# Metronlab/bow

Measured on AMD Instinct MI355X. Metric: rows/sec rolling-mean on 1B-row float64, higher is better.
Workload: dtype f64; 1 GPU; IntervalRolling(interval=10, offset=0)+Aggregate(WindowStart,ArithmeticMean), dense int64 ts=i + float64 u01 values, 1000000000 rows/GPU resident in HBM, null_count=0; rows_per_gpu=1000000000, windows_per_gpu=100000000, parallelism=rows range-partitioned x1

## Files before the change

### bow_amd/capi.py

```python
import contextlib
import ctypes as C
import os

import numpy as np

_HERE = os.path.dirname(os.path.abspath(__file__))
LIB_PATH = os.environ.get("BOWGPU_LIB") or os.path.join(_HERE, "libbowgpu.so")

FLOAT64, INT64, BOOLEAN, STRING = 1, 2, 3, 4
HOST, DEVICE, HOST_PINNED = 0, 1, 2
TYPE_NAMES = {"float64": FLOAT64, "int64": INT64, "bool": BOOLEAN, "utf8": STRING}

AGG = {
    "WindowStart": 0, "Sum": 1, "ArithmeticMean": 2, "Min": 3, "Max": 4, "Count": 5, "First": 6,
    "Last": 7, "IntegralStep": 8, "IntegralTrapezoid": 9, "WeightedAverageStep": 10,
    "WeightedAverageLinear": 11, "NumRows": 12, "Mode": 13,
}
INTERP = {"WindowStart": 0, "Linear": 1, "StepPrevious": 2, "None": 3, "Const": 4}

MAX_FACTORS = 4
CARRY_MAX_AGGS = 16
ABI_VERSION = 7

ERR_NAMES = {
# ... 146 lines not shown
    n = C.c_int(0)
    arr = (C.c_int * 64)()
    check(lib().bowgpu_get_devices(arr, 64, C.byref(n)))
    return [arr[i] for i in range(n.value)]


def fanout_counts():
    a, b = C.c_int64(0), C.c_int64(0)
    check(lib().bowgpu_fanout_counts(C.byref(a), C.byref(b)))
    return a.value, b.value


def last_call_ranks():
    n = C.c_int(0)
    check(lib().bowgpu_last_call_ranks(C.byref(n)))
    return n.value


class devices:

    def __init__(self, ids, min_rows=None):
        self.ids, self.min_rows = list(ids), min_rows

    def __enter__(self):
        self.prev = get_devices()
        set_devices(self.ids, self.min_rows)
        return self

    def __exit__(self, *exc):
        set_devices(self.prev, (1 << 20) if self.min_rows is not None else None)
        return False


def mem_info():
    f, t = C.c_int64(0), C.c_int64(0)
    check(lib().bowgpu_mem_info(C.byref(f), C.byref(t)))
    return f.value, t.value


def trim(all_threads=True):
    n = C.c_int64(0)
    check(lib().bowgpu_trim(1 if all_threads else 0, C.byref(n)))
    return n.value


def check(rc):
    if rc != 0:
        raise BowGpuError(rc, lib().bowgpu_last_error().decode("utf-8", "replace"))


ROUTE_NO_SIMPLE, ROUTE_FORCE_GENERAL, ROUTE_NO_LONG_ONLY, ROUTE_LONG_CLASSIC, ROUTE_LONG_STREAM_ALL = 1, 2, 4, 8, 16
ROUTE_SIMPLE_SMALL_LIST, ROUTE_SIMPLE_LARGE_LIST, ROUTE_TW_F64, ROUTE_SIMPLE_PADDED, ROUTE_INTERP_TILE = 32, 64, 128, 256, 512
ROUTE_PINNED_STAGE, ROUTE_STRICT_ORDER, ROUTE_NO_FUSED, ROUTE_TW_ROWS, ROUTE_INTERP_COPIES = 1024, 2048, 4096, 8192, 16384
ROUTE_QUEUE_HOST, ROUTE_QUEUE_DEVICE = 32768, 65536


def set_route(mask):
    check(lib().bowgpu_debug_set_route(C.c_uint32(mask)))


def get_route():
    m = C.c_uint32(0)
    check(lib().bowgpu_debug_get_route(C.byref(m)))
    return m.value


class route:

    def __init__(self, mask):
        self.mask = mask

    def __enter__(self):
        self.prev = get_route()
        set_route(self.mask)
        return self

    def __exit__(self, *exc):
        set_route(self.prev)
        return False


AGG_ROUTES = (("auto", 0), ("classic-long", ROUTE_LONG_CLASSIC), ("stream-all", ROUTE_LONG_STREAM_ALL),
              ("small-list", ROUTE_SIMPLE_SMALL_LIST), ("large-list", ROUTE_SIMPLE_LARGE_LIST), ("padded", ROUTE_SIMPLE_PADDED), ("tw-rows", ROUTE_TW_ROWS),
              ("queue-device", ROUTE_NO_LONG_ONLY | ROUTE_QUEUE_DEVICE), ("queue-host", ROUTE_NO_LONG_ONLY | ROUTE_QUEUE_HOST),
              ("lean", ROUTE_NO_SIMPLE | ROUTE_NO_LONG_ONLY), ("general", ROUTE_FORCE_GENERAL | ROUTE_NO_LONG_ONLY))
INTERP_ROUTES = (("wave3", 0), ("tile", ROUTE_INTERP_TILE))


def agg_routes():
    for label, mask in AGG_ROUTES:
        with route(mask):
            yield label


class DeviceBuffer:

    def __init__(self, nbytes):
        self.nbytes = int(nbytes)
        p = C.c_void_p()
        check(lib().bowgpu_malloc(C.byref(p), C.c_int64(self.nbytes)))
        self.ptr = p.value

    @classmethod
    def from_numpy(cls, arr):
        arr = np.ascontiguousarray(arr)
        b = cls(max(arr.nbytes, 8))
        if arr.nbytes:
# ... 520 lines not shown
```

### bow_amd/csrc/api.cpp

```cpp

#include <stdarg.h>
#include <stdio.h>
#include <stdlib.h>
#include <string.h>
#include <time.h>
#include <execinfo.h>
#include <signal.h>
#include <unistd.h>

#include <algorithm>
#include <atomic>
#include <condition_variable>
#include <mutex>
#include <thread>
#include <vector>

#include "common.h"

namespace bowgpu {

static thread_local char g_err[512] = "";

void set_error(const char *fmt, ...) {
    va_list ap;
// ... 600 lines not shown
    case BOWGPU_AGG_FIRST:
    case BOWGPU_AGG_LAST: return BOWGPU_INPUT_DEPENDENT;
    case BOWGPU_AGG_MODE: return BOWGPU_INPUT_DEPENDENT;
    default: return BOWGPU_FLOAT64;
    }
}

bool kind_never_nil(int kind) {
    return kind == BOWGPU_AGG_WINDOW_START || kind == BOWGPU_AGG_SUM || kind == BOWGPU_AGG_COUNT || kind == BOWGPU_AGG_NUM_ROWS;
}

bool kind_reads_values(int kind) { return !(kind == BOWGPU_AGG_WINDOW_START || kind == BOWGPU_AGG_NUM_ROWS); }

struct AggRun {
    Plan plan;
    std::vector<DevCol> dcols;
    std::vector<DevOut> douts;
    AggParams params;
    int inclusive = 0;
    int new_interval_col = -1;
};

static int validate_aggs(const bowgpu_col *cols, int32_t ncols, int32_t ts_col, const bowgpu_agg *aggs, int32_t naggs,
                         int *inclusive, int *new_interval_col) {
    if (naggs <= 0) return fail(BOWGPU_ERR_NO_AGG, "at least one column aggregation is required");
    int nic = -1;
    for (int i = 0; i < naggs; i++) {
        if (aggs[i].col < 0 || aggs[i].col >= ncols) return fail(BOWGPU_ERR_BAD_COL, "aggregation %d: no column with index %d", i, aggs[i].col);
        if (aggs[i].kind < 0 || aggs[i].kind >= BOWGPU_AGG__COUNT) return fail(BOWGPU_ERR_ARG, "aggregation %d: unknown kind %d", i, aggs[i].kind);
        if (aggs[i].n_factors < 0 || aggs[i].n_factors > BOWGPU_MAX_FACTORS) return fail(BOWGPU_ERR_ARG, "aggregation %d: bad factor count", i);
        const int t = cols[aggs[i].col].type;
        if (t != BOWGPU_FLOAT64 && t != BOWGPU_INT64)
            return fail(BOWGPU_ERR_UNSUPPORTED, "aggregation %d: column type %d is outside the device path (Float64/Int64 only)", i, t);
        if (kind_needs_inclusive(aggs[i].kind)) *inclusive = 1;
        if (aggs[i].col == ts_col) nic = i;
    }
    if (nic == -1) return fail(BOWGPU_ERR_KEEP_INTERVAL, "must keep interval column");
    *new_interval_col = nic;
    return 0;
}

struct AggJob {
    std::vector<DevCol> dcols;
    std::vector<DevOut> douts;
    DevCol dts;
    AggParams P;
    int64_t W = 0;
    size_t scratch_bytes = 0;
    int inclusive = 0;
    bool counts_used = false;
    bool tail_wrote_host = false;
    bool check_plan = false;
    bool band_rows = false;
};
static thread_local bool g_plan_from_caller = false;
static int64_t compact_long_max_rows(const bowgpu_agg *aggs, int32_t naggs) {
    bool step = false, trap = false, mm = false, fl = false;
    for (int i = 0; i < naggs; i++) {
        const int k = aggs[i].kind;
        step |= k == BOWGPU_AGG_INTEGRAL_STEP || k == BOWGPU_AGG_WAVG_STEP;
        trap |= k == BOWGPU_AGG_INTEGRAL_TRAPEZOID || k == BOWGPU_AGG_WAVG_LINEAR;
        mm |= k == BOWGPU_AGG_MIN || k == BOWGPU_AGG_MAX;
        fl |= k == BOWGPU_AGG_FIRST || k == BOWGPU_AGG_LAST;
    }
    if ((step && trap) || mm) return kCompactLongBothMaxAvgRows;
    if (step || trap || fl) return kCompactLongMaxAvgRows;
    return 0;
}
static thread_local bool g_strict_order = false;

static void pending_drop(Ctx *c);

static int job_build(Ctx *c, const bowgpu_col *cols, int32_t ncols, int32_t ts_col, const Plan &plan, int inclusive,
                     const bowgpu_agg *aggs, int32_t naggs, bowgpu_out *outs, int64_t wid_base, int64_t W,
                     bool holds_row0, AggJob *job, int nullable_per_pass = 4) {
    pending_drop(c);
    const bowgpu_col *tsc = &cols[ts_col];
    const int64_t n = tsc->length;
    for (int i = 0; i < ncols; i++)
        if (cols[i].length != n) return fail(BOWGPU_ERR_ARG, "column %d has %lld rows, interval column has %lld", i, (long long)cols[i].length, (long long)n);

    if (tsc->validity && tsc->null_count != 0) {
        DevCol probe;
        BG_TRY(devcol_prepare(c, tsc, &probe, false, true));
        if (probe.null_count > 0)
            return fail(BOWGPU_ERR_TS_NULLS, "interval column has %lld nulls: outside the device path", (long long)probe.null_count);
    }

    job->dcols.clear();
    job->dcols.resize(ncols);
    job->douts.clear();
    job->douts.resize(naggs);
    job->W = W;
    job->inclusive = inclusive;
    job->check_plan = g_plan_from_caller;
    std::vector<DevCol> &dcols = job->dcols;
    std::vector<int> slot_of(ncols, -1);
    AggParams &P = job->P;
    memset(&P, 0, sizeof P);
    {
        bowgpu_col t = *tsc;
        t.validity = nullptr;
        t.null_count = 0;
        BG_TRY(devcol_prepare(c, &t, &job->dts, true, false));
    }
    P.ts = reinterpret_cast<const int64_t *>(job->dts.values);
// ... 61 lines not shown
        BG_TRY(devout_prepare(c, &outs[i], W, &job->douts[i], i));
        a.out_values = job->douts[i].values;
        a.out_valid = kind_never_nil(aggs[i].kind) ? nullptr : reinterpret_cast<uint32_t *>(job->douts[i].validity);
    }

    P.first_pass_slot = kMaxCols;
    P.last_val_slot = -1;
    for (int i = 0; i < naggs; i++) {
        const AggDesc &d = P.aggs[i];
        const int k = d.kind;
        const int idx = d.slot + 1;
        P.pass_mask[idx] |= 1u << i;
        uint32_t fl = 0;
        if (kind_reads_values(k)) fl |= kPassNeedVals;
        if (k == BOWGPU_AGG_MIN || k == BOWGPU_AGG_MAX) fl |= kPassMinMax;
        if (k == BOWGPU_AGG_FIRST || k == BOWGPU_AGG_LAST) fl |= kPassFirstLast;
        if (d.out_valid) fl |= kPassNullable;
        if (k >= BOWGPU_AGG_INTEGRAL_STEP && k <= BOWGPU_AGG_WAVG_LINEAR && d.slot >= 0) P.cols[d.slot].need_ts = 1;
        P.pass_flags[idx] |= fl;
        if (d.slot < P.first_pass_slot) P.first_pass_slot = d.slot;
        if (kind_reads_values(k) && d.slot > P.last_val_slot) P.last_val_slot = d.slot;
    }
    for (int s = 0; s <= kMaxCols; s++) {
        int nn = 0;
        for (int i = 0; i < naggs; i++) if ((P.pass_mask[s] >> i) & 1u) nn += P.aggs[i].out_valid != nullptr;
        if (nn > P.n_nullable_max) P.n_nullable_max = nn;
    }

    const int64_t ntiles = (n + 511) / 512;
    const int64_t sub_cap = ntiles / kLongLists + 2;
    job->scratch_bytes = 8192 + (size_t)sub_cap * kLongLists * 16;
    void *dscr;
    BG_TRY(ctx_scratch(c, job->scratch_bytes, &dscr));
    P.status = reinterpret_cast<uint32_t *>(dscr);
    P.long_list = reinterpret_cast<int64_t *>(reinterpret_cast<char *>(dscr) + 8192);
    P.long_cap = sub_cap;
    return 0;
}

constexpr size_t kCountsOffset = 1024;
constexpr size_t kReadbackBytes = kCountsOffset + 8 * kMaxAggs;
static_assert(kStatusWords * 4 <= kCountsOffset, "status words overlap the counters");

static void job_bitmaps(AggJob *job, const bowgpu_agg *aggs, int32_t naggs, bool all_ones, BitmapBatch *b) {
    memset(b, 0, sizeof *b);
    b->n = naggs;
    b->status_words = kStatusWords;
    b->nbits = job->W > 0 ? job->W : 0;
    b->status = job->P.status;
    b->counts = reinterpret_cast<unsigned long long *>(reinterpret_cast<char *>(job->P.status) + kCountsOffset);
    for (int i = 0; i < naggs; i++) {
        b->work[i] = reinterpret_cast<uint32_t *>(job->douts[i].validity);
        const bowgpu_out *u = job->douts[i].user;
        b->user[i] = (u && u->residency == BOWGPU_DEVICE) ? u->validity : nullptr;
        b->ones[i] = all_ones || kind_never_nil(aggs[i].kind);
        b->count[i] = !kind_never_nil(aggs[i].kind);
    }
}

static int job_enqueue_tail(Ctx *c, AggJob *job, const bowgpu_agg *aggs, int32_t naggs) {
    const int64_t W = job->W;
    if (W > 0) {
        BitmapBatch b;
        job_bitmaps(job, aggs, naggs, false, &b);
        if (W <= kFinishHostBits) {
            BG_TRY(ctx_pinned(c, 16384, reinterpret_cast<void **>(&b.host_block)));
            job->tail_wrote_host = true;
        } else if (job->counts_used) BG_HIP(hipMemsetAsync(b.counts, 0, 8 * kMaxAggs, c->stream));
        BG_TRY(launch_finish_bitmaps(c, b));
        job->counts_used = true;
    }
    for (int i = 0; i < naggs; i++) BG_TRY(devout_finish(c, &job->douts[i], W, job->P.aggs[i].out_type, 0, false));
    return 0;
}

static int job_readback(Ctx *c, AggJob *job, uint32_t **hstat, uint64_t **hcnt) {
    char *hp;
    BG_TRY(ctx_pinned(c, 16384, reinterpret_cast<void **>(&hp)));
    if (job->tail_wrote_host) job->tail_wrote_host = false;
    else BG_HIP(hipMemcpyAsync(hp, job->P.status, kReadbackBytes, hipMemcpyDeviceToHost, c->stream));
    *hstat = reinterpret_cast<uint32_t *>(hp);
    *hcnt = reinterpret_cast<uint64_t *>(hp + kCountsOffset);
    return 0;
}

static bool simple_applies(const AggJob *job, const bowgpu_agg *aggs, int32_t naggs, const Plan &plan, bool time_weighted, int *need,
                           bool *is_int, bool *has_nulls, bool *wide) {
    const AggParams &P = job->P;
    if ((job->inclusive && !time_weighted) || !P.fits32 || naggs > kSimpleMaxAggs) return false;
    if (P.W <= 0) return false;

    const int64_t slot0_start = P.s0 + (int64_t)((uint64_t)P.wid_base * (uint64_t)P.interval);
    if (plan.first_ts < slot0_start && !(P.pre_rows && P.wid_base == 0)) return false;
    *wide = (uint64_t)plan.last_ts - (uint64_t)slot0_start >= 0xFFFFFFF0ull || P.W >= 0xFFFFFFF0ll;
    *need = 0;
    *is_int = true;
    *has_nulls = false;
    for (int s = 0; s < P.ncols; s++) {
        *has_nulls = *has_nulls || P.cols[s].vbits != nullptr;
        *is_int = P.cols[0].type == BOWGPU_INT64;
    }
    for (int i = 0; i < naggs; i++) {
        const int k = aggs[i].kind;
        if (k >= BOWGPU_AGG_INTEGRAL_STEP && k <= BOWGPU_AGG_WAVG_LINEAR && !time_weighted) return false;
        if (k == BOWGPU_AGG_MIN || k == BOWGPU_AGG_MAX) *need |= 1;
        if (k == BOWGPU_AGG_FIRST || k == BOWGPU_AGG_LAST) *need |= 2;
    }
    if (route_mask() & BOWGPU_ROUTE_NO_SIMPLE) return false;
    return true;
}

static void simple_params_build(const AggJob *job, const bowgpu_agg *aggs, int32_t naggs, bool wide, SimpleParams *out) {
    const AggParams &P = job->P;
    SimpleParams &S = *out;
    memset(&S, 0, sizeof S);
    S.ts = P.ts;
    S.n = P.n; S.interval = P.interval; S.W = P.W;
    S.wid_base = P.wid_base;
    S.magic = P.magic;
    S.s0 = P.s0 + (int64_t)((uint64_t)P.wid_base * (uint64_t)P.interval);
    S.m32 = P.m32; S.sh1 = P.sh1_32; S.sh2 = P.sh2_32;
    S.shift_k = 0;
    if (wide) {
        int k = 0;
        while (k < 31 && !(((uint64_t)P.interval >> k) & 1ull)) k++;
        S.shift_k = k;
        const uint64_t d = (uint64_t)P.interval >> k;
        int l = 0;
        while (l < 32 && (1ull << l) < d) l++;
        S.m32 = (uint32_t)((((1ull << l) - d) << 32) / d) + 1;
        S.sh1 = l < 1 ? (uint32_t)l : 1u;
        S.sh2 = l > 1 ? (uint32_t)(l - 1) : 0u;
    }
    S.naggs = naggs;
    S.ncols = P.ncols > 0 ? P.ncols : 1;
    S.values[0] = P.ts;
    for (int s = 0; s < P.ncols; s++) {
        S.values[s] = P.cols[s].values;
        S.vbits[s] = P.cols[s].vbits; S.vbit0[s] = P.cols[s].vbit0; S.vwords[s] = P.cols[s].vwords;
        S.col_is_int[s] = P.cols[s].type == BOWGPU_INT64;
    }
    for (int i = 0; i < naggs; i++) {
        S.kind[i] = aggs[i].kind;
        S.nfac[i] = aggs[i].n_factors;
        for (int f = 0; f < aggs[i].n_factors && f < BOWGPU_MAX_FACTORS; f++) S.fac[i][f] = aggs[i].factors[f];
        S.col[i] = P.aggs[i].slot < 0 ? 0 : P.aggs[i].slot;
        S.out_values[i] = reinterpret_cast<uint64_t *>(P.aggs[i].out_values);
        S.out_valid[i] = P.aggs[i].out_valid;
    }
    for (int i = 0; i < naggs; i++) {
        const int k = aggs[i].kind;
        if (k == BOWGPU_AGG_INTEGRAL_STEP || k == BOWGPU_AGG_WAVG_STEP) S.need |= kNeedStep;
        if (k == BOWGPU_AGG_INTEGRAL_TRAPEZOID || k == BOWGPU_AGG_WAVG_LINEAR) S.need |= kNeedTrap;
        if (k == BOWGPU_AGG_MIN || k == BOWGPU_AGG_MAX) S.need |= kNeedMinMax;
        if (k == BOWGPU_AGG_SUM || k == BOWGPU_AGG_MEAN) S.need |= kNeedSum;
        if (k == BOWGPU_AGG_FIRST || k == BOWGPU_AGG_LAST) S.need |= kNeedFirstLast;
        const int cls = (k == BOWGPU_AGG_MIN || k == BOWGPU_AGG_MAX) ? 1 : (k == BOWGPU_AGG_INTEGRAL_STEP || k == BOWGPU_AGG_WAVG_STEP) ? 2
                        : (k == BOWGPU_AGG_INTEGRAL_TRAPEZOID || k == BOWGPU_AGG_WAVG_LINEAR) ? 3
                        : (k == BOWGPU_AGG_SUM || k == BOWGPU_AGG_MEAN || k == BOWGPU_AGG_FIRST || k == BOWGPU_AGG_LAST) ? 0 : 4;
        S.kind_mask[cls] |= 1u << i;
        S.col_mask[S.col[i]] |= 1u << i;
    }
    S.status = P.status; S.long_list = P.long_list; S.long_cap = P.long_cap;
    S.inclusive = job->inclusive ? 1 : 0;
    S.pre_rows = P.pre_rows;
    S.unaligned_mask = (reinterpret_cast<uintptr_t>(P.ts) & 15) ? 0x80000000u : 0u;
    for (int s = 0; s < S.ncols; s++)
        if (reinterpret_cast<uintptr_t>(S.values[s]) & 15) S.unaligned_mask |= 1u << s;
}

static int job_launch_tiles(Ctx *c, AggJob *job, const bowgpu_agg *aggs, int32_t naggs, const Plan *plan, bool allow_simple,
                            bool *used_simple, bool force_large_list = false, bool *used_small_list = nullptr) {
    AggParams &P = job->P;
    const int64_t W = job->W;
    *used_simple = false;
    bool small_dummy = false;
    if (!used_small_list) used_small_list = &small_dummy;
    *used_small_list = false;
    if (W <= 0) { BG_HIP(hipMemsetAsync(P.status, 0, kReadbackBytes, c->stream)); return 0; }
    bool lean = !job->inclusive;
    for (int i = 0; i < naggs; i++)
        if (aggs[i].kind >= BOWGPU_AGG_INTEGRAL_STEP && aggs[i].kind <= BOWGPU_AGG_WAVG_LINEAR) lean = false;
    const uint32_t route = route_mask();
    const bool force = (route & BOWGPU_ROUTE_FORCE_GENERAL) != 0;
    if (force) lean = false;
    int need = 0;
    bool is_int = false, has_nulls = false, wide = false;
    bool simple = lean && allow_simple && plan && simple_applies(job, aggs, naggs, *plan, false, &need, &is_int, &has_nulls, &wide);
    const bool tw = !lean && !force && allow_simple && plan &&
                    simple_applies(job, aggs, naggs, *plan, true, &need, &is_int, &has_nulls, &wide);
    simple = simple || tw;
    P.bits_preset = simple ? 1 : 0;
    {
        BitmapBatch b;
        job_bitmaps(job, aggs, naggs, simple, &b);
        if (job->check_plan && plan) { b.check_ts = P.ts; b.check_n = P.n; b.check_first = plan->first_ts; b.check_last = plan->last_ts; }
        BG_TRY(launch_preset_bitmaps(c, b));
        job->counts_used = false;
    }
    BG_HIP(hipEventRecord(c->ev0, c->stream));
    if (simple) {
        SimpleParams S;
        simple_params_build(job, aggs, naggs, wide, &S);
        if (tw) {
            const int64_t lim53 = 1ll << 53;
            const bool ts32 = !wide && !P.pre_rows && plan->first_ts > -lim53 && plan->last_ts < lim53 && S.s0 > -lim53 && !(route & BOWGPU_ROUTE_TW_F64);
            const bool compact = has_nulls && ts32 && !force_large_list && !(route & BOWGPU_ROUTE_TW_ROWS) && P.n / P.W >= kCompactMinAvgRows;
            if (compact) {
                BG_TRY(launch_rolling_twc(c, S, P.n / P.W > 128));
                *used_small_list = true;
                c->last_kernel_name = "rolling_twc_kernel";
            } else {
                BG_TRY(launch_rolling_tw(c, S, is_int, has_nulls, wide, ts32));
                c->last_kernel_name = "rolling_tw_kernel";
            }
        } else if ([&] {
                       const int64_t lim53 = 1ll << 53;
                       const bool ts32 = !wide && !P.pre_rows && plan->first_ts > -lim53 && plan->last_ts < lim53 && S.s0 > -lim53;
                       const bool sums_and_extrema = (S.need & kNeedSum) && (S.need & kNeedMinMax);
                       if (job->band_rows) return false;
                       if (has_nulls && ts32 && !force_large_list && !(route & BOWGPU_ROUTE_TW_ROWS) && P.n / P.W > 128 && P.n / P.W <= compact_long_max_rows(aggs, naggs)) return true;
                       return has_nulls && ts32 && sums_and_extrema && !force_large_list && !(route & BOWGPU_ROUTE_TW_ROWS) && P.n / P.W >= kCompactValuesMinAvgRows;
                   }()) {
            BG_TRY(launch_rolling_twc(c, S, P.n / P.W > 128));
            *used_small_list = true;
            c->last_kernel_name = "rolling_twc_kernel";
        } else {
            const int64_t small_list_rows = rolling_simple_plain(S, is_int, has_nulls) ? 3 : 5;
            const bool dense = force_large_list || ((route & BOWGPU_ROUTE_SIMPLE_LARGE_LIST) ? true : (route & BOWGPU_ROUTE_SIMPLE_SMALL_LIST) ? false : P.n / P.W < small_list_rows);
            *used_small_list = !dense;
            BG_TRY(launch_rolling_simple(c, S, need, is_int, has_nulls, wide, dense));
        }
        *used_simple = true;
    } else if (lean && !P.pre_rows) {
        BG_TRY(launch_rolling_fast(c, P));
        c->last_kernel_name = "rolling_wave_kernel";
    } else {
        static const bool trace = [] { const char *t = getenv("BOWGPU_TRACE_ROUTE"); return t && t[0] == '1'; }();
        if (trace && !force && !(route & BOWGPU_ROUTE_NO_SIMPLE) && allow_simple)
            fprintf(stderr, "bowgpu route: general kernel (n=%lld W=%lld interval=%lld inclusive=%d naggs=%d pre_rows=%lld wid_base=%lld "
                            "fits32=%d allow_simple=%d plan=%d first_ts=%lld s0=%lld)\n", (long long)P.n, (long long)P.W,
                    (long long)P.interval, (int)job->inclusive, naggs, (long long)P.pre_rows, (long long)P.wid_base, (int)P.fits32,
                    (int)allow_simple, plan ? 1 : 0, plan ? (long long)plan->first_ts : 0ll, (long long)P.s0);
        BG_TRY(launch_rolling_aggregate(c, P));
        c->last_kernel_name = "rolling_agg_kernel";
// ... 479 lines not shown
        BG_HIP(hipStreamSynchronize(c->stream));
    }
    return 0;
}

static int run_aggregate(Ctx *c, const bowgpu_col *cols, int32_t ncols, int32_t ts_col, const Plan &plan,
                         int inclusive, const bowgpu_agg *aggs, int32_t naggs, bowgpu_out *outs,
                         int64_t wid_base, int64_t W, int64_t *long_windows, double *kernel_ms) {
    int n_mode = 0;
    for (int i = 0; i < naggs; i++) n_mode += aggs[i].kind == BOWGPU_AGG_MODE;
    if (n_mode > 0 && (wid_base != 0 || W != plan.W)) return fail(BOWGPU_ERR_UNSUPPORTED, "Mode runs on unsharded calls only");
    if (wid_base == 0 && W == plan.W && cols[ts_col].validity && cols[ts_col].null_count != 0 && cols[ts_col].length > 0) {
        DevCol dts;
        BG_TRY(devcol_prepare(c, &cols[ts_col], &dts, true, true));
        if (dts.null_count > 0) return run_aggregate_null_ts(c, cols, ncols, ts_col, plan, inclusive, aggs, naggs, outs, dts, long_windows, kernel_ms);
    }
    if (long_windows) *long_windows = 0;
    if (kernel_ms) *kernel_ms = 0;
    std::vector<std::vector<int>> batches;
    {
        std::vector<int> cur, slot_of(ncols, -1), nullable_in_slot;
        auto flush = [&]() {
            if (!cur.empty()) batches.push_back(cur);
            cur.clear(); nullable_in_slot.clear();
            std::fill(slot_of.begin(), slot_of.end(), -1);
        };
        for (int i = 0; i < naggs; i++) {
            if (aggs[i].kind == BOWGPU_AGG_MODE) continue;
            for (int attempt = 0; attempt < 2; attempt++) {
                bool fits = (int)cur.size() < kMaxAggs;
                int s = -1;
                bool new_slot = false;
                const bool reads = kind_reads_values(aggs[i].kind), nullable = !kind_never_nil(aggs[i].kind);
                if (fits && reads) {
                    s = slot_of[aggs[i].col];
                    if (s >= 0 && nullable && nullable_in_slot[s] >= 4) s = -1;
                    if (s < 0) { new_slot = true; fits = (int)nullable_in_slot.size() < kMaxCols; }
                }
                if (!fits) { flush(); continue; }
                if (reads) {
                    if (new_slot) { s = (int)nullable_in_slot.size(); nullable_in_slot.push_back(0); slot_of[aggs[i].col] = s; }
                    if (nullable) nullable_in_slot[s]++;
                }
                cur.push_back(i);
                break;
            }
        }
        flush();
    }
    for (const std::vector<int> &at : batches) {
        if ((int)at.size() == naggs) {
            AggJob job;
            BG_TRY(job_build(c, cols, ncols, ts_col, plan, inclusive, aggs, naggs, outs, wid_base, W, wid_base == 0, &job));
            BG_TRY(job_run(c, &job, aggs, naggs, long_windows, kernel_ms, true, &plan, true));
            continue;
        }
        std::vector<bowgpu_agg> part;
        std::vector<bowgpu_out> part_outs;
        for (int i : at) { part.push_back(aggs[i]); part_outs.push_back(outs[i]); }
        int64_t lw = 0;
        double ms = 0;
        AggJob job;
        BG_TRY(job_build(c, cols, ncols, ts_col, plan, inclusive, part.data(), (int32_t)part.size(), part_outs.data(), wid_base, W, wid_base == 0, &job));
        BG_TRY(job_run(c, &job, part.data(), (int32_t)part.size(), &lw, &ms, true, &plan, true));
        for (size_t j = 0; j < at.size(); j++) outs[at[j]] = part_outs[j];
        if (long_windows && lw > *long_windows) *long_windows = lw;
        if (kernel_ms) *kernel_ms += ms;
    }
    if (n_mode > 0) return run_modes(c, cols, ncols, ts_col, plan, aggs, naggs, outs, inclusive, long_windows);
    return 0;
}

static int fused_try(Ctx *c, const bowgpu_col *cols, int32_t ncols, int32_t ts_col, const Plan &plan, const bowgpu_options &o, int inclusive,
                     const bowgpu_interp *interps, const bowgpu_agg *aggs, int32_t naggs, bowgpu_out *outs, double *kernel_ms, bool *done) {
    *done = false;
    const bowgpu_col *tsc = &cols[ts_col];
    const int64_t n = tsc->length, W = plan.W;
    if (route_mask() & (BOWGPU_ROUTE_NO_FUSED | BOWGPU_ROUTE_NO_SIMPLE | BOWGPU_ROUTE_FORCE_GENERAL)) return 0;
    if (n <= 0 || W <= 0 || inclusive || o.inclusive || naggs > kSimpleMaxAggs) return 0;
    if (tsc->validity && tsc->null_count != 0) return 0;
    const int64_t lim53 = 1ll << 53;
    if (plan.first_ts < plan.s0 || plan.last_ts >= lim53 || plan.s0 <= -lim53) return 0;
    if (plan.s0 <= -1 && (uint64_t)(-1 - plan.s0) % (uint64_t)plan.interval == 0 && (int64_t)((uint64_t)(-1 - plan.s0) / (uint64_t)plan.interval) < W) return 0;
    if (((uint64_t)plan.interval >> 32) != 0 || (uint64_t)plan.last_ts - (uint64_t)plan.s0 >= 0xFFFFFFF0ull || W >= 0xFFFFFFF0ll) return 0;
    if (n / W < 4 || n / W > 128) return 0;
    for (int i = 0; i < ncols; i++) {
        const int k = interps[i].kind;
        if (k != BOWGPU_INTERP_WINDOW_START && k != BOWGPU_INTERP_LINEAR && k != BOWGPU_INTERP_STEP_PREVIOUS && k != BOWGPU_INTERP_NONE) return 0;
    }
    if (interps[ts_col].kind != BOWGPU_INTERP_WINDOW_START) return 0;
    {
        std::vector<int> used(ncols, 0);
        int distinct = 0;
        for (int i = 0; i < naggs; i++) {
            const int k = aggs[i].kind;
            if ((k >= BOWGPU_AGG_INTEGRAL_STEP && k <= BOWGPU_AGG_WAVG_LINEAR) || k == BOWGPU_AGG_MODE) return 0;
            if (kind_reads_values(k) && !used[aggs[i].col]++) distinct++;
        }
        if (distinct > kMaxCols) return 0;
    }
    AggJob job;
    BG_TRY(job_build(c, cols, ncols, ts_col, plan, 0, aggs, naggs, outs, 0, W, true, &job, kMaxAggs));
    AggParams &P = job.P;
    int need = 0;
    bool is_int = false, has_nulls = false, wide = false;
    if (P.pre_rows || !simple_applies(&job, aggs, naggs, plan, false, &need, &is_int, &has_nulls, &wide) || wide) return 0;
    P.bits_preset = 1;
    {
        BitmapBatch b;
        job_bitmaps(&job, aggs, naggs, true, &b);
        BG_TRY(launch_preset_bitmaps(c, b));
        job.counts_used = false;
    }
    FusedParams F;
    memset(&F, 0, sizeof F);
    simple_params_build(&job, aggs, naggs, false, &F.s);
// ... 906 lines not shown
```

### bow_amd/csrc/common.h

```cpp
#pragma once

#include <hip/hip_runtime.h>
#include <stdint.h>

#include <string>

#include "../../include/bowgpu.h"
#include "debug_routes.h"

namespace bowgpu {

void set_error(const char *fmt, ...);
int fail(int code, const char *fmt, ...);
int hip_fail(hipError_t e, const char *what);

#define BG_HIP(expr)                                         \
    do {                                                     \
        hipError_t _e = (expr);                              \
        if (_e != hipSuccess) return hip_fail(_e, #expr);    \
    } while (0)

#define BG_TRY(expr)              \
    do {                          \
        int _rc = (expr);         \
// ... 35 lines not shown
        uint64_t gen = 0, gen0 = 0;
        uint64_t epoch = 0;
        int64_t s0 = 0, W = 0, first_ts = 0, last_ts = 0, offset_norm = 0, kq = -1, drop = 0, M = 0, wbase = 0;
        int kq_empty = 0, inclusive = 0, e0 = 0;
    } interp_cache;
    void *d_params = nullptr;
    void *null_ts_cache = nullptr;
    void (*null_ts_cache_free)(void *) = nullptr;
};
void ctx_drop_null_ts_cache(Ctx *c);
int ctx_get(Ctx **out);
int ctx_scratch(Ctx *c, size_t bytes, void **dptr);
int ctx_pinned(Ctx *c, size_t bytes, void **hptr);
int ctx_params(Ctx *c, void **dptr);
int ctx_pool(Ctx *c, int slot, size_t bytes, void **dptr);

void devbuf_release(void *p, size_t cap);
void devbuf_cache_drop();
int devbuf_acquire(size_t n, void **p, size_t *cap);
struct DevBuf {
    void *p = nullptr;
    size_t bytes = 0;
    size_t cap = 0;
    DevBuf() = default;
    DevBuf(const DevBuf &) = delete;
    DevBuf &operator=(const DevBuf &) = delete;
    DevBuf(DevBuf &&o) noexcept : p(o.p), bytes(o.bytes), cap(o.cap) { o.p = nullptr; o.bytes = 0; o.cap = 0; }
    DevBuf &operator=(DevBuf &&o) noexcept {
        if (this != &o) { if (p) devbuf_release(p, cap); p = o.p; bytes = o.bytes; cap = o.cap; o.p = nullptr; o.bytes = 0; o.cap = 0; }
        return *this;
    }
    ~DevBuf() { if (p) devbuf_release(p, cap); }
    int alloc(size_t n);
};

struct DevCol {
    const void *values = nullptr;
    const uint32_t *vbits = nullptr;
    int64_t vbit0 = 0;
    int64_t vwords = 0;
    int64_t length = 0;
    int64_t null_count = 0;
    int32_t type = 0;
    DevBuf own_values, own_validity;
};
int devcol_prepare(Ctx *c, const bowgpu_col *col, DevCol *out, bool need_values, bool need_validity);
int count_nulls_device(Ctx *c, DevCol *dc);

struct DevOut {
    void *values = nullptr;
    uint8_t *validity = nullptr;
    int64_t capacity = 0;
    int pool_slot = -1;
    DevBuf own_values, own_validity;
    bowgpu_out *user = nullptr;
};
int copy_d2h(Ctx *c, void *dst, const void *src, size_t bytes, bool registered = false);
int copy_h2d(Ctx *c, void *dst, const void *src, size_t bytes, bool registered = false);
int devout_prepare(Ctx *c, bowgpu_out *out, int64_t slots, DevOut *d, int pool_slot = -1);
int devout_finish(Ctx *c, DevOut *d, int64_t slots, int32_t type, int64_t null_count, bool copy_bitmap = true);

struct MagicDiv {
    uint64_t m;
    uint32_t sh1, sh2;
};
MagicDiv magic_make(uint64_t d);

struct Plan {
    int64_t interval = 0;
    int64_t offset = 0;
    int64_t s0 = 0;
    int64_t W = 0;
    int64_t first_ts = 0, last_ts = 0;
    MagicDiv magic{};
};
int plan_make(Ctx *c, const bowgpu_col *ts, int64_t interval, int64_t raw_offset, Plan *p);
bool kind_needs_inclusive(int kind);
int kind_type(int kind);
bool kind_never_nil(int kind);
bool kind_reads_values(int kind);

int multi_aggregate(const bowgpu_col *cols, int32_t ncols, int32_t ts_col, const Plan &plan, int opt_inclusive, bool strict,
                    const bowgpu_agg *aggs, int32_t naggs, bowgpu_out *outs, bowgpu_agg_info *info, bool *done);
int multi_interpolate_aggregate(const bowgpu_col *cols, int32_t ncols, int32_t ts_col, const Plan &plan, int opt_inclusive, bool strict,
                                const bowgpu_interp *interps, int32_t ninterps, const bowgpu_agg *aggs, int32_t naggs, bowgpu_out *outs,
                                bowgpu_agg_info *info, bool *done);

constexpr int kMaxCols = 8;
constexpr int kMaxAggs = 16;

struct AggDesc {
    int32_t kind;
    int32_t slot;
    int32_t out_type;
    int32_t n_factors;
    double factors[BOWGPU_MAX_FACTORS];
    void *out_values;
    uint32_t *out_valid;
};

struct ColDesc {
    const void *values;
    const uint32_t *vbits;
    int64_t vbit0;
    int64_t vwords;
    int32_t type;
// ... 71 lines not shown
    int64_t prev_v_i64;
};
struct FusedParams {
    SimpleParams s;
    FusedCol cols[kMaxCols];
    double inv_interval;
};
int launch_rolling_fused(Ctx *c, const FusedParams &fp, int need, bool has_nulls);
int interp_validate(const bowgpu_col *cols, int32_t ncols, int32_t ts_col, const bowgpu_options *o, const bowgpu_interp *interps, int32_t ninterps);

int launch_rolling_twc(Ctx *c, const SimpleParams &p, bool long_halo = false);
constexpr int64_t kCompactLongMaxAvgRows = 255;
constexpr int64_t kCompactLongBothMaxAvgRows = 176;
constexpr int64_t kCompactValuesMinAvgRows = 48;
constexpr int64_t kCompactMinAvgRows = 12;
int launch_rolling_aggregate(Ctx *c, const AggParams &p);
int launch_rolling_fast(Ctx *c, const AggParams &p);
constexpr int kLongChunkRows = 4096;
constexpr int kLongStreamRows = 512;
constexpr int64_t kLongOnlyAvgRows = 128;
constexpr int64_t kLongStreamAnyAvgRows = 129;
constexpr int64_t kLongBisectAvgRows = 512;
constexpr int64_t kLongClassicAvgRows = 1ll << 22;
constexpr int kLongLists = 64;
constexpr int kLongCountWord = 16;
constexpr int kStatusWords = kLongCountWord + kLongLists;
struct LongListStarts { int64_t start[kLongLists + 1]; };
size_t long_entry_size();
size_t long_part_size();
int stream_rw_run(Ctx *c, const void *a, const void *b, int64_t bytes_each, void *o0, void *o1, int64_t rows_per_slot, int64_t nslots, bool nt,
                  int reps, float *ms);
int stream_sum_run(Ctx *c, const void *a, const void *b, int64_t bytes_each, int mode, int blocks_per_cu, int reps, uint64_t *d_out, float *ms);
int launch_long_windows_v2(Ctx *c, const AggParams &p, const LongListStarts *starts, void *entries, int32_t *nchunks, int64_t *offsets,
                           int64_t *block_sums, int64_t *d_total, int32_t *work_entry, void *partials, int64_t max_work, bool strict = false,
                           int64_t n_given = 0);
int launch_long_queue(Ctx *c, const AggParams &p, int64_t capacity, void *big_entries, int32_t *big_nchunks, int64_t walk_max_rows, bool strict);
constexpr int kQueueBigWord = 8;
constexpr int64_t kQueueWalkMaxRows = 1024;
size_t long_stream_workspace(int64_t n, int64_t W, int ncols);
int launch_long_stream(Ctx *c, const AggParams &p, void *workspace);
int launch_fix_tail_bits(Ctx *c, uint8_t *bitmap, int64_t nbits);
struct BitmapBatch {
    int32_t n, status_words;
    int64_t nbits;
    uint32_t *work[kMaxAggs];
    uint8_t *user[kMaxAggs];
    int32_t ones[kMaxAggs];
    int32_t count[kMaxAggs];
    uint32_t *status;
    unsigned long long *counts;
    char *host_block;
    const int64_t *check_ts;
    int64_t check_n, check_first, check_last;
};
constexpr int64_t kFinishHostBits = 262144;
int launch_preset_bitmaps(Ctx *c, const BitmapBatch &b);
int launch_finish_bitmaps(Ctx *c, const BitmapBatch &b);
int launch_popcount(Ctx *c, const uint32_t *words, int64_t bit0, int64_t nbits, uint64_t *d_count);
int launch_fetch_two(Ctx *c, const int64_t *col, int64_t i0, int64_t i1, int64_t *host_out);

int launch_mode(Ctx *c, const int64_t *ts, const int64_t *first_idx, int64_t n, int64_t s0, int64_t interval, int64_t W, int pre_rows,
                int inclusive, const void *values,
                const uint32_t *vbits, int64_t vbit0, int is_int, const bowgpu_agg *agg, void *out_values, uint32_t *out_valid,
                int64_t *n_mid, int64_t *n_long);

struct NbrIndex {
    const int64_t *prev_before;
    const int64_t *next_after;
    int64_t g0;
};
int launch_ts_nullfill(Ctx *c, const int64_t *ts, const uint32_t *tbits, int64_t tbit0, int64_t n, const struct NbrIndex &ix, int64_t s0, int64_t interval,
                       const MagicDiv &magic, int inclusive, int64_t *ts_eff, uint64_t *keep, uint64_t *plain, unsigned long long *d_dropped);
struct QuirkFixAgg {
    const void *values; const uint32_t *vbits; int64_t vbit0;
    uint64_t *out_values; uint32_t *out_valid;
    int32_t type, kind, n_factors, _pad;
    double factors[BOWGPU_MAX_FACTORS];
};
struct QuirkFix { int32_t naggs, _pad; QuirkFixAgg a[8]; };
int launch_ts_quirk_fix(Ctx *c, const int64_t *ts, const uint32_t *tbits, int64_t tbit0, int64_t n, const struct NbrIndex &ix, int64_t s0, int64_t interval,
                        const MagicDiv &magic, int64_t W, const QuirkFix &fx, unsigned long long *d_fixed);
int launch_count_to_f64(Ctx *c, uint64_t *v, int64_t n);
int fetch_valid(Ctx *c, const bowgpu_col *col, int64_t row, int *valid);
constexpr int kMaxCompactCols = 16;
struct CompactCols {
    int32_t ncols, ts_col;
    const uint64_t *values[kMaxCompactCols]; const uint32_t *vbits[kMaxCompactCols]; int64_t vbit0[kMaxCompactCols];
    uint64_t *out_values[kMaxCompactCols];
    uint64_t *lookup_bits[kMaxCompactCols];
    uint64_t *patch_values[kMaxCompactCols]; uint32_t *patch_valid[kMaxCompactCols];
    uint64_t *ts_bits;
};
struct PatchInterps {
    int64_t m;
    const uint64_t *both_bits[kMaxCompactCols];
    NbrIndex nbr[kMaxCompactCols];
    int32_t type[kMaxCompactCols], kind[kMaxCompactCols], has_prev[kMaxCompactCols], prev_t_valid[kMaxCompactCols], prev_v_valid[kMaxCompactCols];
    double const_value[kMaxCompactCols], prev_t[kMaxCompactCols], prev_v[kMaxCompactCols];
    int64_t prev_v_i64[kMaxCompactCols];
};
int launch_keep_counts(Ctx *c, const uint64_t *keep, int64_t nw, int32_t *counts);
int launch_compact_rows(Ctx *c, const uint64_t *keep, const int64_t *base, int64_t n, const int64_t *ts_eff, const uint32_t *tbits, int64_t tbit0,
                        const uint64_t *plain, const CompactCols &cc, int64_t *marker, uint32_t *flags);
int launch_pack_flags(Ctx *c, const uint32_t *flags, int64_t m, const CompactCols &cc, uint64_t *marker_bits);
int launch_interp_patch(Ctx *c, const int64_t *marker_out, const uint32_t *marker_valid, int64_t m_out, const uint32_t *flags, const CompactCols &cc,
                        const PatchInterps &px);
// ... 133 lines not shown
```

### bow_amd/csrc/debug_routes.h

```cpp
#pragma once
enum {
    BOWGPU_ROUTE_NO_SIMPLE = 1,
    BOWGPU_ROUTE_FORCE_GENERAL = 2,
    BOWGPU_ROUTE_NO_LONG_ONLY = 4,
    BOWGPU_ROUTE_LONG_CLASSIC = 8,
    BOWGPU_ROUTE_LONG_STREAM_ALL = 16,
    BOWGPU_ROUTE_SIMPLE_SMALL_LIST = 32,
    BOWGPU_ROUTE_SIMPLE_LARGE_LIST = 64,
    BOWGPU_ROUTE_TW_F64 = 128,
    BOWGPU_ROUTE_SIMPLE_PADDED = 256,
    BOWGPU_ROUTE_INTERP_TILE = 512,
    BOWGPU_ROUTE_NO_FUSED = 4096,
    BOWGPU_ROUTE_TW_ROWS = 8192,
    BOWGPU_ROUTE_INTERP_COPIES = 16384,
    BOWGPU_ROUTE_QUEUE_HOST = 32768,
    BOWGPU_ROUTE_QUEUE_DEVICE = 65536,
    BOWGPU_ROUTE__ALL = 131071
};
```

### bow_amd/csrc/rolling_agg.hip

```cpp

#include "agg_device.h"

namespace bowgpu {

namespace {

constexpr int kBlock = 256;
constexpr int kTile = 2048;
constexpr int kHalo = 128;
constexpr int kRows = kTile + kHalo;
constexpr int kChunks = kTile / (2 * kBlock);
constexpr int kCnt = kChunks * 4 + 1;
constexpr int kSpanBits = 2048 + 64;
constexpr int kSpanWords = kSpanBits / 32;
constexpr int kMaxNullable = 8;
constexpr int kGapInline = 4;
constexpr int kGapList = 64;

struct TileShared {
    uint64_t val[kRows];
    uint32_t seg_wid[kRows + 2];
    uint16_t seg_row[kRows + 2];
    uint32_t vbits[kRows / 32 + 2];
    uint32_t obits[kMaxNullable][kSpanWords];
// ... 329 lines not shown
            }
        }
        first_pass = false;
    }
}

__global__ void fix_tail_bits_kernel(uint8_t *bitmap, int64_t nbits) {
    if (threadIdx.x == 0 && blockIdx.x == 0 && (nbits & 7)) bitmap[nbits >> 3] &= (uint8_t)((1u << (nbits & 7)) - 1u);
}

__global__ __launch_bounds__(256) void popcount_kernel(const uint32_t *words, int64_t bit0, int64_t nbits,
                                                       unsigned long long *out) {
    const int64_t w0 = bit0 >> 5, w1 = (bit0 + nbits + 31) >> 5;
    unsigned long long acc = 0;
    for (int64_t w = w0 + blockIdx.x * (int64_t)blockDim.x + threadIdx.x; w < w1; w += (int64_t)gridDim.x * blockDim.x) {
        uint32_t x = words[w];
        const int64_t lo = w << 5;
        if (lo < bit0) x &= ~0u << (bit0 - lo);
        if (lo + 32 > bit0 + nbits) { const int keep = (int)(bit0 + nbits - lo); x &= keep >= 32 ? ~0u : ((1u << keep) - 1u); }
        acc += __popc(x);
    }
    for (int o = 32; o > 0; o >>= 1) acc += __shfl_down(acc, o);
    __shared__ unsigned long long part[4];
    if ((threadIdx.x & 63) == 0) part[threadIdx.x >> 6] = acc;
    __syncthreads();
    if (threadIdx.x == 0) {
        const unsigned long long t = part[0] + part[1] + part[2] + part[3];
        if (t) atomicAdd(out, t);
    }
}

int launch_rolling_aggregate(Ctx *c, const AggParams &p) {
    if (p.n <= 0) return 0;
    const int64_t ntiles = (p.n + kTile - 1) / kTile;
    const int64_t per_xcd = (ntiles + 7) / 8;
    const int64_t grid = per_xcd * 8;
    if (grid > 0x7FFFFFFFll) return fail(BOWGPU_ERR_UNSUPPORTED, "too many rows for one launch: %lld", (long long)p.n);
    bool with_ts = false;
    for (int a = 0; a < p.naggs; a++) with_ts |= (p.aggs[a].kind >= BOWGPU_AGG_INTEGRAL_STEP && p.aggs[a].kind <= BOWGPU_AGG_WAVG_LINEAR);
    if (with_ts) hipLaunchKernelGGL(rolling_agg_kernel<true>, dim3((unsigned)grid), dim3(kBlock), 0, c->stream, p, ntiles, per_xcd);
    else hipLaunchKernelGGL(rolling_agg_kernel<false>, dim3((unsigned)grid), dim3(kBlock), 0, c->stream, p, ntiles, per_xcd);
    BG_HIP(hipGetLastError());
    return 0;
}

__global__ __launch_bounds__(256) void preset_bitmaps_kernel(const BitmapBatch b) {
    const int a = blockIdx.y;
    if (a == 0 && blockIdx.x == 0) {
        for (int i = threadIdx.x; i < b.status_words; i += blockDim.x)
            b.status[i] = (i == 6 && b.check_ts && b.check_n > 0 && (b.check_ts[0] != b.check_first || b.check_ts[b.check_n - 1] != b.check_last)) ? 1u : 0u;
        if (threadIdx.x < kMaxAggs) b.counts[threadIdx.x] = 0ull;
    }
    if (a >= b.n) return;
    const int64_t nwords = (b.nbits + 31) >> 5;
    const uint32_t fill = b.ones[a] ? 0xFFFFFFFFu : 0u;
    uint32_t *w = b.work[a];
    for (int64_t i = (int64_t)blockIdx.x * blockDim.x + threadIdx.x; i < nwords; i += (int64_t)gridDim.x * blockDim.x) {
        uint32_t x = fill;
        if (i == nwords - 1 && (b.nbits & 31)) x &= (1u << (b.nbits & 31)) - 1u;
        w[i] = x;
    }
}
__global__ __launch_bounds__(256) void finish_bitmaps_kernel(const BitmapBatch b) {
    const int a = blockIdx.y;
    if (a >= b.n) return;
    const int64_t nwords = (b.nbits + 31) >> 5, nbytes = (b.nbits + 7) >> 3;
    const uint32_t *w = b.work[a];
    uint8_t *u = b.user[a];
    const bool aligned = (reinterpret_cast<uintptr_t>(u) & 3) == 0;
    unsigned long long acc = 0;
    const bool vec = (reinterpret_cast<uintptr_t>(w) & 15) == 0 && (!u || (reinterpret_cast<uintptr_t>(u) & 15) == 0);
    const int64_t nvec = vec ? ((b.nbits >> 5) >> 2) : 0;
    const int64_t stride = (int64_t)gridDim.x * blockDim.x;
    int64_t g = (int64_t)blockIdx.x * blockDim.x + threadIdx.x;
    for (; g + 3 * stride < nvec; g += 4 * stride) {
        const uint4 *q = reinterpret_cast<const uint4 *>(w) + g;
        const uint4 x0 = q[0], x1 = q[stride], x2 = q[2 * stride], x3 = q[3 * stride];
        if (b.count[a]) acc += __popc(x0.x) + __popc(x0.y) + __popc(x0.z) + __popc(x0.w) + __popc(x1.x) + __popc(x1.y) + __popc(x1.z) + __popc(x1.w) +
                               __popc(x2.x) + __popc(x2.y) + __popc(x2.z) + __popc(x2.w) + __popc(x3.x) + __popc(x3.y) + __popc(x3.z) + __popc(x3.w);
        if (u) {
            uint4 *d = reinterpret_cast<uint4 *>(u) + g;
            d[0] = x0; d[stride] = x1; d[2 * stride] = x2; d[3 * stride] = x3;
        }
    }
    for (; g < nvec; g += stride) {
        const uint4 x = reinterpret_cast<const uint4 *>(w)[g];
        if (b.count[a]) acc += __popc(x.x) + __popc(x.y) + __popc(x.z) + __popc(x.w);
        if (u) reinterpret_cast<uint4 *>(u)[g] = x;
    }
    for (int64_t i = 4 * nvec + (int64_t)blockIdx.x * blockDim.x + threadIdx.x; i < nwords; i += (int64_t)gridDim.x * blockDim.x) {
        uint32_t x = w[i];
        if (i == nwords - 1 && (b.nbits & 31)) x &= (1u << (b.nbits & 31)) - 1u;
        if (b.count[a]) acc += __popc(x);
        if (u) {
            if (aligned && 4 * i + 4 <= nbytes) reinterpret_cast<uint32_t *>(u)[i] = x;
            else for (int k = 0; k < 4 && 4 * i + k < nbytes; k++) u[4 * i + k] = (uint8_t)(x >> (8 * k));
        }
    }
    if (b.count[a]) {
        __shared__ unsigned long long wave_sum[4];
        for (int o = 32; o > 0; o >>= 1) acc += __shfl_down(acc, o);
        if ((threadIdx.x & 63) == 0) wave_sum[threadIdx.x >> 6] = acc;
        __syncthreads();
        if (threadIdx.x == 0) {
            const unsigned long long t = wave_sum[0] + wave_sum[1] + wave_sum[2] + wave_sum[3];
            if (b.host_block) reinterpret_cast<unsigned long long *>(b.host_block + 1024)[a] = t;
            else if (t) atomicAdd(&b.counts[a], t);
        }
    } else if (b.host_block && threadIdx.x == 0) reinterpret_cast<unsigned long long *>(b.host_block + 1024)[a] = 0;
    if (b.host_block && a == 0 && blockIdx.x == 0)
        for (int t = threadIdx.x; t < b.status_words; t += blockDim.x) reinterpret_cast<uint32_t *>(b.host_block)[t] = b.status[t];
}

static unsigned bitmap_grid(int64_t nbits) {
    const int64_t nwords = (nbits + 31) >> 5;
    int64_t g = (nwords + 255) / 256;
    return (unsigned)(g < 1 ? 1 : g > 1024 ? 1024 : g);
}
int launch_preset_bitmaps(Ctx *c, const BitmapBatch &b) {
    hipLaunchKernelGGL(preset_bitmaps_kernel, dim3(bitmap_grid(b.nbits), b.n > 0 ? b.n : 1), dim3(256), 0, c->stream, b);
    BG_HIP(hipGetLastError());
    return 0;
}
int launch_finish_bitmaps(Ctx *c, const BitmapBatch &b) {
    if (b.n <= 0 || b.nbits <= 0) return 0;
    hipLaunchKernelGGL(finish_bitmaps_kernel, dim3(b.host_block ? 1u : bitmap_grid(b.nbits), b.n), dim3(256), 0, c->stream, b);
    BG_HIP(hipGetLastError());
    return 0;
}

int launch_fix_tail_bits(Ctx *c, uint8_t *bitmap, int64_t nbits) {
    if ((nbits & 7) == 0) return 0;
    hipLaunchKernelGGL(fix_tail_bits_kernel, dim3(1), dim3(64), 0, c->stream, bitmap, nbits);
    BG_HIP(hipGetLastError());
    return 0;
}

__global__ void fetch_two_kernel(const int64_t *col, int64_t i0, int64_t i1, int64_t *host_out) {
    if (threadIdx.x == 0) host_out[0] = col[i0];
    if (threadIdx.x == 1) host_out[1] = col[i1];
}
int launch_fetch_two(Ctx *c, const int64_t *col, int64_t i0, int64_t i1, int64_t *host_out) {
    hipLaunchKernelGGL(fetch_two_kernel, dim3(1), dim3(64), 0, c->stream, col, i0, i1, host_out);
    BG_HIP(hipGetLastError());
    return 0;
}

int launch_popcount(Ctx *c, const uint32_t *words, int64_t bit0, int64_t nbits, uint64_t *d_count) {
    BG_HIP(hipMemsetAsync(d_count, 0, 8, c->stream));
    if (nbits <= 0) return 0;
    const int64_t nwords = (nbits + 63) / 32;
    int64_t grid = (nwords + 255) / 256;
    if (grid > 512) grid = 512;
    hipLaunchKernelGGL(popcount_kernel, dim3((unsigned)grid), dim3(256), 0, c->stream, words, bit0, nbits,
                       reinterpret_cast<unsigned long long *>(d_count));
    BG_HIP(hipGetLastError());
    return 0;
}

}
```

Baseline: 315.2 billion rows/s.

## Write validity bitmaps in place and fold finish-bitmap readback into one kernel

When the simple tile path runs and the user output lives on device, validity bits are written directly into the user's bitmap, so the later copy from the scratch bitmap is skipped. The finish kernel now only launches grid rows for aggregates that need counting or copying, and writes counts and status straight to pinned host memory using an atomic ticket scheme. This avoids a separate memset and device-to-host copy for large bitmaps. The preset kernel is also vectorized to 16-byte stores. The old chained path stays available behind a debug route flag. The ticket protocol adds atomics and complexity, and in-place writes depend on the alignment checks being correct.

```diff
diff --git a/bow_amd/capi.py b/bow_amd/capi.py
--- a/bow_amd/capi.py
+++ b/bow_amd/capi.py
@@ -222,7 +222,7 @@
 ROUTE_NO_SIMPLE, ROUTE_FORCE_GENERAL, ROUTE_NO_LONG_ONLY, ROUTE_LONG_CLASSIC, ROUTE_LONG_STREAM_ALL = 1, 2, 4, 8, 16
 ROUTE_SIMPLE_SMALL_LIST, ROUTE_SIMPLE_LARGE_LIST, ROUTE_TW_F64, ROUTE_SIMPLE_PADDED, ROUTE_INTERP_TILE = 32, 64, 128, 256, 512
 ROUTE_PINNED_STAGE, ROUTE_STRICT_ORDER, ROUTE_NO_FUSED, ROUTE_TW_ROWS, ROUTE_INTERP_COPIES = 1024, 2048, 4096, 8192, 16384
-ROUTE_QUEUE_HOST, ROUTE_QUEUE_DEVICE = 32768, 65536
+ROUTE_QUEUE_HOST, ROUTE_QUEUE_DEVICE, ROUTE_BITMAP_CHAIN = 32768, 65536, 131072
 
 
 def set_route(mask):
diff --git a/bow_amd/csrc/api.cpp b/bow_amd/csrc/api.cpp
--- a/bow_amd/csrc/api.cpp
+++ b/bow_amd/csrc/api.cpp
@@ -676,6 +676,7 @@
     bool tail_wrote_host = false;
     bool check_plan = false;
     bool band_rows = false;
+    bool in_place_ok = false;
 };
 static thread_local bool g_plan_from_caller = false;
 static int64_t compact_long_max_rows(const bowgpu_agg *aggs, int32_t naggs) {
@@ -843,7 +844,7 @@
     for (int i = 0; i < naggs; i++) {
         b->work[i] = reinterpret_cast<uint32_t *>(job->douts[i].validity);
         const bowgpu_out *u = job->douts[i].user;
-        b->user[i] = (u && u->residency == BOWGPU_DEVICE) ? u->validity : nullptr;
+        b->user[i] = (u && u->residency == BOWGPU_DEVICE && !job->douts[i].in_place) ? u->validity : nullptr;
         b->ones[i] = all_ones || kind_never_nil(aggs[i].kind);
         b->count[i] = !kind_never_nil(aggs[i].kind);
     }
@@ -854,12 +855,12 @@
     if (W > 0) {
         BitmapBatch b;
         job_bitmaps(job, aggs, naggs, false, &b);
-        if (W <= kFinishHostBits) {
+        if (W <= kFinishHostBits || !(route_mask() & BOWGPU_ROUTE_BITMAP_CHAIN)) {
             BG_TRY(ctx_pinned(c, 16384, reinterpret_cast<void **>(&b.host_block)));
             job->tail_wrote_host = true;
         } else if (job->counts_used) BG_HIP(hipMemsetAsync(b.counts, 0, 8 * kMaxAggs, c->stream));
         BG_TRY(launch_finish_bitmaps(c, b));
-        job->counts_used = true;
+        job->counts_used = !b.host_block;
     }
     for (int i = 0; i < naggs; i++) BG_TRY(devout_finish(c, &job->douts[i], W, job->P.aggs[i].out_type, 0, false));
     return 0;
@@ -958,6 +959,18 @@
     S.unaligned_mask = (reinterpret_cast<uintptr_t>(P.ts) & 15) ? 0x80000000u : 0u;
     for (int s = 0; s < S.ncols; s++)
         if (reinterpret_cast<uintptr_t>(S.values[s]) & 15) S.unaligned_mask |= 1u << s;
+}
+
+static void job_place_bitmaps(AggJob *job, bool wave_tiles) {
+    const bool on = wave_tiles && job->in_place_ok && !(route_mask() & BOWGPU_ROUTE_BITMAP_CHAIN) && job->W > 0 && (((job->W + 7) >> 3) & 3) == 0;
+    for (size_t i = 0; i < job->douts.size(); i++) {
+        DevOut &d = job->douts[i];
+        const bowgpu_out *u = d.user;
+        if (!d.work) d.work = d.validity;
+        d.in_place = on && u && u->residency == BOWGPU_DEVICE && !(reinterpret_cast<uintptr_t>(u->validity) & 3);
+        d.validity = d.in_place ? u->validity : d.work;
+        if (job->P.aggs[i].out_valid) job->P.aggs[i].out_valid = reinterpret_cast<uint32_t *>(d.validity);
+    }
 }
 
 static int job_launch_tiles(Ctx *c, AggJob *job, const bowgpu_agg *aggs, int32_t naggs, const Plan *plan, bool allow_simple,
@@ -982,6 +995,7 @@
                     simple_applies(job, aggs, naggs, *plan, true, &need, &is_int, &has_nulls, &wide);
     simple = simple || tw;
     P.bits_preset = simple ? 1 : 0;
+    job_place_bitmaps(job, simple);
     {
         BitmapBatch b;
         job_bitmaps(job, aggs, naggs, simple, &b);
@@ -1567,6 +1581,7 @@
         if ((int)at.size() == naggs) {
             AggJob job;
             BG_TRY(job_build(c, cols, ncols, ts_col, plan, inclusive, aggs, naggs, outs, wid_base, W, wid_base == 0, &job));
+            job.in_place_ok = wid_base == 0;
             BG_TRY(job_run(c, &job, aggs, naggs, long_windows, kernel_ms, true, &plan, true));
             continue;
         }
@@ -1577,6 +1592,7 @@
         double ms = 0;
         AggJob job;
         BG_TRY(job_build(c, cols, ncols, ts_col, plan, inclusive, part.data(), (int32_t)part.size(), part_outs.data(), wid_base, W, wid_base == 0, &job));
+        job.in_place_ok = wid_base == 0;
         BG_TRY(job_run(c, &job, part.data(), (int32_t)part.size(), &lw, &ms, true, &plan, true));
         for (size_t j = 0; j < at.size(); j++) outs[at[j]] = part_outs[j];
         if (long_windows && lw > *long_windows) *long_windows = lw;
diff --git a/bow_amd/csrc/common.h b/bow_amd/csrc/common.h
--- a/bow_amd/csrc/common.h
+++ b/bow_amd/csrc/common.h
@@ -111,6 +111,8 @@
     uint8_t *validity = nullptr;
     int64_t capacity = 0;
     int pool_slot = -1;
+    uint8_t *work = nullptr;
+    bool in_place = false;
     DevBuf own_values, own_validity;
     bowgpu_out *user = nullptr;
 };
@@ -288,6 +290,8 @@
     char *host_block;
     const int64_t *check_ts;
     int64_t check_n, check_first, check_last;
+    int32_t ny;
+    int32_t idx[kMaxAggs];
 };
 constexpr int64_t kFinishHostBits = 262144;
 int launch_preset_bitmaps(Ctx *c, const BitmapBatch &b);
diff --git a/bow_amd/csrc/debug_routes.h b/bow_amd/csrc/debug_routes.h
--- a/bow_amd/csrc/debug_routes.h
+++ b/bow_amd/csrc/debug_routes.h
@@ -15,5 +15,6 @@
     BOWGPU_ROUTE_INTERP_COPIES = 16384,
     BOWGPU_ROUTE_QUEUE_HOST = 32768,
     BOWGPU_ROUTE_QUEUE_DEVICE = 65536,
-    BOWGPU_ROUTE__ALL = 131071
+    BOWGPU_ROUTE_BITMAP_CHAIN = 131072,
+    BOWGPU_ROUTE__ALL = 262143
 };
diff --git a/bow_amd/csrc/rolling_agg.hip b/bow_amd/csrc/rolling_agg.hip
--- a/bow_amd/csrc/rolling_agg.hip
+++ b/bow_amd/csrc/rolling_agg.hip
@@ -405,18 +405,23 @@
         if (threadIdx.x < kMaxAggs) b.counts[threadIdx.x] = 0ull;
     }
     if (a >= b.n) return;
-    const int64_t nwords = (b.nbits + 31) >> 5;
+    const int64_t nwords = (b.nbits + 31) >> 5, full = b.nbits >> 5;
     const uint32_t fill = b.ones[a] ? 0xFFFFFFFFu : 0u;
     uint32_t *w = b.work[a];
-    for (int64_t i = (int64_t)blockIdx.x * blockDim.x + threadIdx.x; i < nwords; i += (int64_t)gridDim.x * blockDim.x) {
+    const int64_t lead = (int64_t)(((16u - (uint32_t)(reinterpret_cast<uintptr_t>(w) & 15)) & 15) >> 2);
+    const int64_t head = lead < full ? lead : full;
+    const int64_t nvec = (full - head) >> 2;
+    const int64_t tid = (int64_t)blockIdx.x * blockDim.x + threadIdx.x, nthr = (int64_t)gridDim.x * blockDim.x;
+    uint4 *q = reinterpret_cast<uint4 *>(w + head);
+    for (int64_t i = tid; i < nvec; i += nthr) q[i] = make_uint4(fill, fill, fill, fill);
+    if (tid < head) w[tid] = fill;
+    for (int64_t i = head + 4 * nvec + tid; i < nwords; i += nthr) {
         uint32_t x = fill;
         if (i == nwords - 1 && (b.nbits & 31)) x &= (1u << (b.nbits & 31)) - 1u;
         w[i] = x;
     }
 }
-__global__ __launch_bounds__(256) void finish_bitmaps_kernel(const BitmapBatch b) {
-    const int a = blockIdx.y;
-    if (a >= b.n) return;
+__device__ __forceinline__ unsigned long long finish_one_bitmap(const BitmapBatch &b, int a) {
     const int64_t nwords = (b.nbits + 31) >> 5, nbytes = (b.nbits + 7) >> 3;
     const uint32_t *w = b.work[a];
     uint8_t *u = b.user[a];
@@ -450,19 +455,39 @@
             else for (int k = 0; k < 4 && 4 * i + k < nbytes; k++) u[4 * i + k] = (uint8_t)(x >> (8 * k));
         }
     }
-    if (b.count[a]) {
+    return acc;
+}
+__global__ __launch_bounds__(256) void finish_bitmaps_kernel(const BitmapBatch b) {
+    const int a = (int)blockIdx.y < b.ny ? b.idx[blockIdx.y] : -1;
+    const bool counted = a >= 0 && b.count[a];
+    unsigned long long acc = a >= 0 ? finish_one_bitmap(b, a) : 0ull;
+    unsigned long long t = 0;
+    if (counted) {
         __shared__ unsigned long long wave_sum[4];
         for (int o = 32; o > 0; o >>= 1) acc += __shfl_down(acc, o);
         if ((threadIdx.x & 63) == 0) wave_sum[threadIdx.x >> 6] = acc;
         __syncthreads();
-        if (threadIdx.x == 0) {
-            const unsigned long long t = wave_sum[0] + wave_sum[1] + wave_sum[2] + wave_sum[3];
-            if (b.host_block) reinterpret_cast<unsigned long long *>(b.host_block + 1024)[a] = t;
-            else if (t) atomicAdd(&b.counts[a], t);
-        }
-    } else if (b.host_block && threadIdx.x == 0) reinterpret_cast<unsigned long long *>(b.host_block + 1024)[a] = 0;
-    if (b.host_block && a == 0 && blockIdx.x == 0)
-        for (int t = threadIdx.x; t < b.status_words; t += blockDim.x) reinterpret_cast<uint32_t *>(b.host_block)[t] = b.status[t];
+        t = wave_sum[0] + wave_sum[1] + wave_sum[2] + wave_sum[3];
+    }
+    unsigned long long *host_counts = reinterpret_cast<unsigned long long *>(b.host_block + 1024);
+    if (!b.host_block) {
+        if (threadIdx.x == 0 && t) atomicAdd(&b.counts[a], t);
+    } else if (gridDim.x == 1) {
+        if (threadIdx.x == 0 && a >= 0) host_counts[a] = t;
+        if (blockIdx.y == 0)
+            for (int s = threadIdx.x; s < b.status_words; s += blockDim.x) reinterpret_cast<uint32_t *>(b.host_block)[s] = b.status[s];
+    } else {
+        constexpr int kTicketShift = 44;
+        if (threadIdx.x == 0 && counted) {
+            const unsigned long long before = atomicAdd(&b.counts[a], (1ull << kTicketShift) + t);
+            if ((before >> kTicketShift) == gridDim.x - 1) {
+                host_counts[a] = (before + t) & ((1ull << kTicketShift) - 1);
+                atomicExch(&b.counts[a], 0ull);
+            }
+        }
+        if (blockIdx.x == 0 && blockIdx.y == 0)
+            for (int s = threadIdx.x; s < b.status_words; s += blockDim.x) reinterpret_cast<uint32_t *>(b.host_block)[s] = b.status[s];
+    }
 }
 
 static unsigned bitmap_grid(int64_t nbits) {
@@ -475,9 +500,16 @@
     BG_HIP(hipGetLastError());
     return 0;
 }
-int launch_finish_bitmaps(Ctx *c, const BitmapBatch &b) {
-    if (b.n <= 0 || b.nbits <= 0) return 0;
-    hipLaunchKernelGGL(finish_bitmaps_kernel, dim3(b.host_block ? 1u : bitmap_grid(b.nbits), b.n), dim3(256), 0, c->stream, b);
+int launch_finish_bitmaps(Ctx *c, const BitmapBatch &b0) {
+    if (b0.n <= 0 || b0.nbits <= 0) return 0;
+    BitmapBatch b = b0;
+    b.ny = 0;
+    for (int a = 0; a < b.n; a++)
+        if (b.count[a] || b.user[a]) b.idx[b.ny++] = a;
+    if (b.ny == 0 && !b.host_block) return 0;
+    unsigned gx = b.ny == 0 || (b.host_block && b.nbits <= kFinishHostBits) ? 1u : bitmap_grid(b.nbits);
+    if (b.host_block && gx > 256) gx = 256;
+    hipLaunchKernelGGL(finish_bitmaps_kernel, dim3(gx, b.ny > 0 ? b.ny : 1), dim3(256), 0, c->stream, b);
     BG_HIP(hipGetLastError());
     return 0;
 }
```

Measured after the change: 318.0 billion rows/s (median of 6 runs). No clear change (+0.9%).
